# mlnoga/nightlight

Hardware: AMD Instinct MI355X
Metric: stacked Mpixels/sec (sigma-clip, 128x4096x4096 fp32) (higher is better)
Workload: dtype f32; 1 GPU; 128 x 4096x4096 fp32 frames, sigma-clip kappa=3, rows split over 1 GPU(s), frames resident in HBM; frames=128, width=4096, image_rows=4096, rows_per_gpu=4096, mode=2, preheat_steps=64, clip_low=6836157, clip_high=13270993

## Files before the change

### nightlight_amd/csrc/nlstack_internal.hpp

```cpp
#pragma once

#include <string.h>

#include <string>
#include <vector>

#include "background.hpp"
#include "dev_memory.hpp"
#include "stars.hpp"
#include "stack_kernels.h"

namespace nl {

extern thread_local std::string g_err;
int fail(int code, const char *fmt, ...);

int require_device(int *count = nullptr);
int select_device(int device);

template <class Run>
int with_scratch_handle(int width, int height, int device, Run run)
{
    nl_stack_t *h = nl_stack_create(1, width, height, 0, height, device);
    if (!h) return NL_ERR_HIP;
// ... 13 lines not shown
        hipError_t e_ = (call);                                                             \
        if (e_ != hipSuccess)                                                               \
            return fail(NL_ERR_HIP, "%s failed: %s (%s:%d)", #call, hipGetErrorString(e_), \
                        __FILE__, __LINE__);                                                \
    } while (0)

constexpr int kTimingRing = 64;
constexpr int kStageSlots = 4;
constexpr int kStatBlocks = 2048;
constexpr int kOrderRing = 8;
constexpr size_t kScratchBytes = sizeof(unsigned long long) * nl::kScratchWords;

struct nl_stack {
    int device = 0;
    int n_frames = 0, width = 0, height = 0, row0 = 0, rows = 0;
    int n_capacity = 0;
    int64_t npix = 0;
    int64_t fstride = 0;
    int64_t fstride_owned = 0;
    hipStream_t stream = nullptr;
    hipEvent_t ring_start[kTimingRing] = {}, ring_stop[kTimingRing] = {};
    hipEvent_t ring_dom0[kTimingRing] = {}, ring_dom1[kTimingRing] = {};
    bool ring_dom0_is_start[kTimingRing] = {};
    bool ring_timed[kTimingRing] = {};
    int64_t pass_seq = 0;
    int64_t copy_waits_pass = 0;
    hipEvent_t ev_start = nullptr, ev_stop = nullptr;
    hipEvent_t ev_dom0 = nullptr, ev_dom1 = nullptr;
    hipStream_t side_stream = nullptr;
    hipEvent_t ev_fork = nullptr, ev_join = nullptr;
    hipEvent_t ev_order[kOrderRing] = {};
    int order_seq = 0;
    unsigned ev_rel = 0;
    float *d_frames_owned = nullptr;
    float *d_frames = nullptr;
    float *d_out = nullptr;
    float *d_acc = nullptr;
    float *d_weights = nullptr;
    bool has_weights = false;
    float *d_xstat = nullptr;
    unsigned long long *d_sets = nullptr;
    int cur_set = 0;
    bool sets_clean = false;
    bool partial_clean = false;
    unsigned long long *d_partial = nullptr;
    float2 *d_bounds = nullptr;
    unsigned char *d_nrounds = nullptr;
    bool bounds_tried = false;
    unsigned fb_hint = 0;
    unsigned gen_hint = 0;
    bool last_weighted = false;
    bool last_fused = false;
    bool last_tail_fused = false;
    bool last_lists = false;
    unsigned dev_flags = 0;
    unsigned *d_fb_list = nullptr;
    unsigned *d_fb_count = nullptr;
    unsigned *d_gen_list = nullptr;
    bool force_exact = false;
    int exact_flavour = 0;
    bool last_used_fast = false;
    unsigned long long *d_counters = nullptr;
    unsigned long long *d_counters_own = nullptr;
    double *d_stat_partial = nullptr;
    unsigned *d_lf_list[2] = {nullptr, nullptr};
    uint4 *d_lf_state[2] = {nullptr, nullptr};
    unsigned *d_lf_count = nullptr;
    int lf_lanes = 0;
    bool lf_tried = false;
    nl::DevBuffer ingest;
    hipStream_t copy_stream = nullptr;
    size_t stage_cap[kStageSlots] = {0, 0, 0, 0};
    nl::DevBuffer ingest_async;
    double *d_stat_partial_async = nullptr;
    void *h_stage[kStageSlots] = {nullptr, nullptr, nullptr, nullptr};
    hipEvent_t stage_done[kStageSlots] = {nullptr, nullptr, nullptr, nullptr};
    bool stage_used[kStageSlots] = {false, false, false, false};
    int stage_next = 0;
    bool uploads_pending = false;
    struct FrameScratch {
        nl::ParkedBuffer bp_diff, bp_seg, bp_list;
        nl::DevBuffer bp_small;
        nl::DevBuffer cfa;
        nl::StarWork star_work;
        nl::BackWork back_work;
        size_t bytes() const
        {
            return bp_diff.bytes + bp_seg.bytes + bp_list.bytes + bp_small.bytes + cfa.bytes + star_work.bytes() +
                   back_work.bytes();
        }
        void release(int device)
        {
            bp_diff.release(device);
            bp_seg.release(device);
            bp_list.release(device);
            bp_small.release();
            cfa.release();
            star_work.release();
            back_work.release();
        }
    } frame_scratch;
    int max_grid = 0;
    int last_mode = -1;
    bool last_has_counters = false;
    bool pending = false;
    const char *last_kernel = "";
// ... 16 lines not shown
```

### nightlight_amd/csrc/nlstack_pass.hip

```cpp
#include <mutex>

#include "nlstack_internal.hpp"

namespace {

constexpr int kListGrid = 2048;
constexpr int kCoopGrid = 16384;
constexpr int kListLanes = 4;
constexpr unsigned kFusedMaxList = 512;
constexpr unsigned kTailFusedMaxList = 512;
constexpr const char *kWinsorPlanShallow = "1:6,1:12:4,0:0:4";
constexpr const char *kWinsorPlanDeep = "2:12,2:16:8,3:24:4,0:0:4";
constexpr int kWinsorCascadeMaxFrames = 96;

constexpr unsigned kDevPlainProtocol = 1u;
constexpr unsigned kDevReplayInFront = 2u;
constexpr unsigned kDevNoDecision = 4u;
constexpr unsigned kDevNoTile = 16u;
constexpr unsigned kDevUntimed = 32u;
constexpr unsigned kDevNoWinsorCascade = 128u;
constexpr unsigned kDevNoSharedHints = 512u;
constexpr unsigned kDevRemovedPasses = 1024u | 2048u;
constexpr unsigned kDevTwoStreamTail = 8192u;
constexpr unsigned kDevNoCertificate = 16384u;

struct HintKey { int frames; int64_t npix; int mode; bool weighted; };
struct HintEntry { HintKey key; unsigned fb, gen; };
std::mutex g_hint_mu;
std::vector<HintEntry> g_hints;
constexpr size_t kHintEntries = 32;

void hints_store(const HintKey &k, unsigned fb, unsigned gen)
{
    std::lock_guard<std::mutex> lk(g_hint_mu);
    for (HintEntry &e : g_hints)
        if (e.key.frames == k.frames && e.key.npix == k.npix && e.key.mode == k.mode && e.key.weighted == k.weighted) {
            e.fb = fb; e.gen = gen;
            return;
        }
    if (g_hints.size() >= kHintEntries) g_hints.erase(g_hints.begin());
    g_hints.push_back({k, fb, gen});
}

bool hints_load(const HintKey &k, unsigned *fb, unsigned *gen)
{
    std::lock_guard<std::mutex> lk(g_hint_mu);
    for (const HintEntry &e : g_hints)
        if (e.key.frames == k.frames && e.key.npix == k.npix && e.key.mode == k.mode && e.key.weighted == k.weighted) {
            *fb = e.fb; *gen = e.gen;
            return true;
        }
    return false;
}

int next_pow2(int n)
{
    int p = 1;
    while (p < n) p <<= 1;
    return p;
}

}

static int dense_grid(int64_t items, int64_t max_grid, int width, int pixels_per_item)
{
    int64_t g = items < max_grid ? items : max_grid;
    if (g <= 8 || items <= g) return (int)g;
    g &= ~(int64_t)7;
    auto gcd = [](int64_t x, int64_t y) { while (y) { const int64_t t = x % y; x = y; y = t; } return x; };
    const int64_t most = (int64_t)width / 64 > 8 * pixels_per_item ? (int64_t)width / 64 : 8 * pixels_per_item;
    for (int tries = 0; tries < 64 && g > 8 && gcd(g * pixels_per_item, (int64_t)width) > most; tries++) g -= 8;
    return (int)g;
}

extern "C" {

static const nl::LinfitCascade *linfit_cascade(nl_stack_t *h, nl::LinfitCascade *out)
// ... 31 lines not shown
    if (h->d_bounds) return true;
    if (h->bounds_tried) return false;
    h->bounds_tried = true;
    if (cached_malloc((void **)&h->d_bounds, (size_t)nl::kBoundRounds * (size_t)h->npix * sizeof(float2), h->device) != hipSuccess ||
        cached_malloc((void **)&h->d_nrounds, (size_t)h->npix, h->device) != hipSuccess) {
        (void)hipGetLastError();
        if (h->d_bounds) { (void)hipFree(h->d_bounds); h->d_bounds = nullptr; }
        h->d_nrounds = nullptr;
        return false;
    }
    return true;
}

static bool fused_protocol_on()
{
    static const bool on = [] { const char *e = getenv("NL_FUSED"); return !(e && e[0] == '0'); }();
    return on;
}

static int auto_select_mode(int l)
{
    if (l >= 25) return NL_ST_LINEAR_FIT;
    if (l >= 15) return NL_ST_WINSOR_SIGMA;
    if (l >= 6) return NL_ST_SIGMA;
    return NL_ST_MEAN;
}


enum class Engine {
    Mean,
    MedianRegisters,
    MedianMultiLane,
    Listed,
    SigmaFast,
    WeightedTile,
    DenseReplay,
    ExactColumns,
};

struct PassSetup {
    int mode;
    bool weighted;
    bool timed;
    bool fused;
    nl::StackArgs a;
};

struct PassFacts {
    bool has_counters = false;
    bool used_fast = false;
    bool lists = false;
    bool fused = false;
    bool tail_fused = false;
    bool zeroed_behind = false;
};

static void set_last_pass(nl_stack *h, const PassFacts &f)
{
    h->last_has_counters = f.has_counters;
    h->last_used_fast = f.used_fast;
    h->last_lists = f.lists;
    h->last_fused = f.fused;
    h->last_tail_fused = f.tail_fused;
    h->sets_clean = f.fused;
}

static Engine select_engine(const nl_stack *h, int mode, bool weighted, const nl::StackArgs &a)
{
    const bool fast = !h->force_exact;
    const int n = a.n_frames;
    if (mode == NL_ST_MEAN) return Engine::Mean;
    if (fast && mode == NL_ST_MEDIAN && nl::fast_supported(mode, weighted, n, a.npix)) return Engine::MedianRegisters;
    if (fast && mode == NL_ST_MEDIAN && nl::fast_ml_supported(mode, weighted, n, a.npix)) return Engine::MedianMultiLane;
    if (fast && h->d_fb_list &&
        (nl::mad_fast_supported(mode, weighted, n, a.npix) || (mode == NL_ST_MAD_SIGMA && nl::fast_ml_supported(mode, weighted, n, a.npix)) ||
         nl::linfit_ml_supported(mode, n, a.npix) || nl::linfit_fast_supported(mode, n, a.npix)))
        return Engine::Listed;
    if (fast && h->d_fb_list && (nl::fast_supported(mode, weighted, n, a.npix) || nl::fast_ml_supported(mode, weighted, n, a.npix)))
        return Engine::SigmaFast;
    if ((h->exact_flavour == 3 ||
         (fast && weighted && !(h->dev_flags & kDevNoTile) &&
          n <= (mode == NL_ST_WINSOR_SIGMA ? nl::kTileMaxFramesWinsor : nl::kTileMaxFramesSigma))) &&
        nl::tile_supported(mode, weighted, n))
        return Engine::WeightedTile;
    if ((h->exact_flavour == 2 || (fast && (weighted || n > 512))) && nl::coop_supported(mode, weighted, n))
        return Engine::DenseReplay;
    return Engine::ExactColumns;
}

static nl::FastArgs list_args(const nl_stack *h, bool exact_list, bool generic_list)
{
    nl::FastArgs f;
    memset(&f, 0, sizeof f);
    if (exact_list) {
        f.fb_list = h->d_fb_list;
        f.fb_count = h->d_fb_count;
        f.fb_capacity = (unsigned)h->npix;
    }
    if (generic_list) {
        f.gen_list = h->d_gen_list;
        f.gen_count = h->d_fb_count + 1;
        f.gen_capacity = (unsigned)h->npix;
    }
    return f;
}

static int replay_list(nl_stack *h, int mode, bool weighted, const nl::StackArgs &a)
{
    int lanes = 0;
    size_t lds = 0;
    if (nl::exact_plan(mode, weighted, a.n_frames, a.n_pad, kListLanes, &lanes, &lds) != 0)
        return fail(NL_ERR_TOO_MANY_FRAMES, "%d frames do not fit the per-pixel LDS column (mode %d)", a.n_frames, mode);
    nl::StackArgs e = a;
    e.list = h->d_fb_list;
    e.list_count = h->d_fb_count;
    e.list_capacity = (unsigned)h->npix;
// ... 117 lines not shown
        unsigned *base = reinterpret_cast<unsigned *>(cb.state[i]);
        f.cas_list[i] = base;
        f.cas_state[i] = base + 2 * (size_t)h->npix;
        f.cas_count[i] = cb.list[i];
    }
    f.cas_stages = pl.stages;
    for (int k = 0; k < pl.stages; k++) { f.cas_pass[k] = pl.pass[k]; f.cas_cap[k] = pl.cap[k]; f.cas_group[k] = pl.group[k]; }
    return true;
}

static int run_sigma_fast(nl_stack *h, const PassSetup &p, PassFacts *facts)
{
    const int mode = p.mode;
    nl::StackArgs a = p.a;
    if (mode == NL_ST_WINSOR_SIGMA && a.n_frames > 128 && fused_protocol_on() && ensure_bounds(h)) {
        a.bounds = h->d_bounds;
        a.nrounds = h->d_nrounds;
    }
    nl::FastArgs f = list_args(h, true, true);
    f.fb_snap = h->d_fb_count + 2;
    f.gen_hint = h->gen_hint;
    const bool cascade = mode == NL_ST_WINSOR_SIGMA && winsor_setup(h, a.n_frames, f);
    nl::StackArgs e = a;
    e.list = h->d_fb_list;
    e.list_count = h->d_fb_count;
    e.list_capacity = (unsigned)h->npix;
    const bool coop = nl::coop_supported(mode, p.weighted, a.n_frames) != 0;
    unsigned *snap = h->d_fb_count + 2;
    int grid0 = 0, grid1 = 0;
    replay_grids(h, &grid0, &grid1);
    struct Fork { nl_stack *h; nl::StackArgs e; int mode; unsigned *snap; int grid0; bool cascade; hipError_t err; } fork{h, e, mode, snap, grid0, cascade, hipSuccess};
    nl::AfterDominant after = nullptr;
    if (coop) after = [](void *u) {
        Fork *k = static_cast<Fork *>(u);
        nl_stack *hh = k->h;
        const char *ignored = "";
        const bool own = (hh->dev_flags & kDevUntimed) || k->cascade;
        hipEvent_t fork_ev = own ? hh->ev_fork : hh->ev_dom1;
        hipError_t err = own ? hipEventRecord(hh->ev_fork, hh->stream) : hipSuccess;
        const bool in_front = (hh->dev_flags & kDevReplayInFront) != 0;
        const hipStream_t s = in_front ? hh->stream : hh->side_stream;
        if (!in_front && err == hipSuccess) err = hipStreamWaitEvent(hh->side_stream, fork_ev, 0);
        nl::StackArgs first = k->e;
        first.list_snap = k->snap;
        first.list_part = 0;
        if (err == hipSuccess) err = nl::launch_stack_sigma_coop(k->mode, first, k->grid0, s, &ignored);
        if (err == hipSuccess) err = hipEventRecord(hh->ev_join, s);
        k->err = err;
    };
    static const bool tail_fused_on = [] { const char *e = getenv("NL_TAIL_FUSED"); return !(e && e[0] == '0'); }();
    const bool tail_fused = tail_fused_on && !(h->dev_flags & (kDevTwoStreamTail | kDevReplayInFront)) && p.fused && coop && !cascade &&
                            nl::tail_fused_supported(mode, p.weighted, a.n_frames) != 0 && h->fb_hint != 0 &&
                            h->fb_hint - 1u <= kTailFusedMaxList;
    nl::StackArgs first_replay = e;
    first_replay.list_snap = snap;
    first_replay.list_part = 0;
    unsigned replay_blocks = h->fb_hint + 31u;
    replay_blocks = replay_blocks < 64u ? 64u : replay_blocks > 768u ? 768u : replay_blocks;
    if (tail_fused) after = nullptr;
    if (a.n_frames <= 128)
        NL_HIP(nl::launch_stack_sigma_fast(a, f, h->stream, &h->last_kernel, p.timed ? h->ev_dom1 : nullptr,
                                           mode == NL_ST_WINSOR_SIGMA, after, &fork,
                                           tail_fused ? &first_replay : nullptr, replay_blocks));
    else
        NL_HIP(nl::launch_stack_sigma_ml(a, f, h->stream, &h->last_kernel, p.timed ? h->ev_dom1 : nullptr,
                                         mode == NL_ST_WINSOR_SIGMA, after, &fork));
    NL_HIP(fork.err);
    if (coop) {
        const char *exact_name = "";
        e.list_snap = snap;
        e.list_part = 1;
        NL_HIP(nl::launch_stack_sigma_coop(mode, e, grid1, h->stream, &exact_name));
        if (!tail_fused) NL_HIP(hipStreamWaitEvent(h->stream, h->ev_join, 0));
    } else {
        const int rc = replay_list(h, mode, p.weighted, a);
        if (rc != NL_OK) return rc;
    }
    if (!p.fused) {
        NL_HIP(nl::launch_reduce_counters(h->d_partial, nl::kClipSlots, h->d_counters, h->stream, h->d_fb_count, true));
        facts->zeroed_behind = true;
    }
    facts->has_counters = true;
    facts->used_fast = true;
    facts->lists = true;
    facts->fused = p.fused;
    facts->tail_fused = tail_fused;
    return NL_OK;
}

static int run_weighted_tile(nl_stack *h, const PassSetup &p, PassFacts *facts)
{
    const int64_t tiles = (p.a.npix + 63) / 64;
    const int64_t g = tiles < (1 << 20) ? tiles : (1 << 20);
    NL_HIP(nl::launch_stack_sigma_tile(p.mode, p.a, (int)g, h->stream, &h->last_kernel));
    NL_HIP(hipEventRecord(h->ev_dom1, h->stream));
    NL_HIP(nl::launch_reduce_counters(h->d_partial, nl::kClipSlots, h->d_counters, h->stream));
    facts->has_counters = true;
    return NL_OK;
}

static int run_dense_replay(nl_stack *h, const PassSetup &p, PassFacts *facts)
{
    nl::StackArgs a = p.a;
    const int rc = decision_pass(h, p, a);
    if (rc != NL_OK) return rc;
    const int per_item = p.mode == NL_ST_MEDIAN ? 1 : nl::coop_group(a);
    const int64_t items = a.npix / per_item;
    const int64_t most = 262144;
    const int g = dense_grid(items, most, h->width, per_item);
    if (p.mode == NL_ST_MEDIAN) NL_HIP(nl::launch_stack_median_coop(a, (int)g, h->stream, &h->last_kernel));
    else                        NL_HIP(nl::launch_stack_sigma_coop(p.mode, a, (int)g, h->stream, &h->last_kernel));
    NL_HIP(hipEventRecord(h->ev_dom1, h->stream));
    NL_HIP(nl::launch_reduce_counters(h->d_partial, nl::kClipSlots, h->d_counters, h->stream));
    facts->has_counters = p.mode != NL_ST_MEDIAN;
    return NL_OK;
}

static int run_exact_columns(nl_stack *h, const PassSetup &p, PassFacts *facts)
{
    nl::StackArgs a = p.a;
    int lanes = 0;
    size_t lds = 0;
    if (nl::exact_plan(p.mode, p.weighted, a.n_frames, a.n_pad, 64, &lanes, &lds) != 0)
        return fail(NL_ERR_TOO_MANY_FRAMES, "%d frames do not fit the per-pixel LDS column (mode %d)", a.n_frames, p.mode);
    a.tiles = (a.npix + lanes - 1) / lanes;
    const int grid = (int)(a.tiles < (int64_t)h->max_grid ? a.tiles : (int64_t)h->max_grid);
    NL_HIP(nl::launch_stack_exact(p.mode, p.weighted, a, lanes, grid, lds, h->stream, &h->last_kernel));
    NL_HIP(hipEventRecord(h->ev_dom1, h->stream));
    NL_HIP(nl::launch_reduce_counters(h->d_partial, nl::kClipSlots, h->d_counters, h->stream));
    facts->has_counters = p.mode != NL_ST_MEDIAN;
    return NL_OK;
}

static int run_async_impl(nl_stack_t *h, int mode, float sigma_low, float sigma_high, float ref_loc);

int nl_stack_run_async(nl_stack_t *h, int mode, float sigma_low, float sigma_high, float ref_loc)
{
    const int rc = run_async_impl(h, mode, sigma_low, sigma_high, ref_loc);
    if (rc != NL_OK && h && h->stream) {
// ... 139 lines not shown
    if (hipSetDevice(h->device) != hipSuccess || hipEventSynchronize(to) != hipSuccess ||
        hipEventElapsedTime(&ms, from, to) != hipSuccess)
        return -1.0f;
    return ms;
}

float nl_stack_last_dominant_kernel_ms(nl_stack_t *h) { return h && h->ev_dom0 ? elapsed_ms(h, h->ev_dom0, h->ev_dom1) : -1.0f; }

int nl_stack_set_exact(nl_stack_t *h, int on)
{
    NL_CHECK_HANDLE(h);
    if (on < 0 || on > 4) return fail(NL_ERR_INVALID_ARG, "set_exact: unknown flavour %d (0 ... 4)", on);
    if (on == 4)
        return fail(NL_ERR_INVALID_ARG, "set_exact: flavour 4 (four pixels per wave) was removed with the experiments build");
    h->force_exact = on != 0;
    h->exact_flavour = on;
    return NL_OK;
}

int nl_stack_set_dev_flags(nl_stack_t *h, unsigned flags)
{
    NL_CHECK_HANDLE(h);
    if (flags & kDevRemovedPasses)
        return fail(NL_ERR_INVALID_ARG, "set_dev_flags: switches 1024 / 2048 (split / persistent LDS-column pass) were removed with the "
                                        "experiments build");
    h->dev_flags = flags;
    return NL_OK;
}

static int64_t last_list_length(nl_stack_t *h, int which)
{
    if (hipSetDevice(h->device) != hipSuccess) return -1;
    if (h->last_lists) {
        unsigned long long c = 0;
        if (hipMemcpyAsync(&c, h->d_counters + 2, sizeof c, hipMemcpyDeviceToHost, h->stream) != hipSuccess) return -1;
        if (hipStreamSynchronize(h->stream) != hipSuccess) return -1;
        return which == 0 ? (int64_t)(c & 0xffffffffull) : (int64_t)(c >> 32);
    }
    unsigned c = 0;
    if (hipMemcpyAsync(&c, h->d_fb_count + which, sizeof c, hipMemcpyDeviceToHost, h->stream) != hipSuccess) return -1;
    if (hipStreamSynchronize(h->stream) != hipSuccess) return -1;
    return (int64_t)c;
}

int64_t nl_stack_last_fallback_pixels(nl_stack_t *h)
{
    if (!h || !h->last_used_fast || !h->d_fb_count) return 0;
    return last_list_length(h, 0);
}

int nl_stack_last_pass_protocol(nl_stack_t *h)
{
    if (!h) return 0;
    return (h->last_fused ? 1 : 0) | (h->last_tail_fused ? 2 : 0);
}

int64_t nl_stack_last_generic_pixels(nl_stack_t *h)
{
    if (!h || !h->last_used_fast || !h->d_fb_count || !h->d_gen_list) return 0;
    return last_list_length(h, 1);
}

int nl_stack_linfit_stage_counts(nl_stack_t *h, unsigned *counts, int n)
{
    if (!h || !counts || n <= 0 || !h->d_lf_count || h->last_mode != NL_ST_LINEAR_FIT || !h->last_used_fast) return 0;
    if (hipSetDevice(h->device) != hipSuccess) return -1;
    unsigned c[nl::kLinfitCounters] = {};
    if (hipMemcpyAsync(c, h->d_lf_count, sizeof c, hipMemcpyDeviceToHost, h->stream) != hipSuccess) return -1;
    if (hipStreamSynchronize(h->stream) != hipSuccess) return -1;
    const int m = n < nl::kLinfitCounters ? n : nl::kLinfitCounters;
    for (int i = 0; i < m; i++) counts[i] = c[i];
    return m;
}

int nl_stack_pass_times(nl_stack_t *h, int back, float *pass_ms, float *dominant_ms)
{
    NL_CHECK_HANDLE(h);
    if (back < 0 || back >= kTimingRing || (int64_t)back >= h->pass_seq)
        return fail(NL_ERR_INVALID_ARG, "pass_times: pass %d back is not in the ring of %d", back, kTimingRing);
    const int slot = (int)((h->pass_seq - 1 - back) % kTimingRing);
    if (!h->ring_timed[slot])
        return fail(NL_ERR_INVALID_ARG, "pass_times: pass %d back ran without timing events (developer switch 32)", back);
    NL_HIP(hipEventSynchronize(h->ring_stop[slot]));
    float ms = -1.0f;
    if (pass_ms) {
        NL_HIP(hipEventElapsedTime(&ms, h->ring_start[slot], h->ring_stop[slot]));
        *pass_ms = ms;
    }
    if (dominant_ms) {
        NL_HIP(hipEventElapsedTime(&ms, h->ring_dom0_is_start[slot] ? h->ring_start[slot] : h->ring_dom0[slot], h->ring_dom1[slot]));
        *dominant_ms = ms;
    }
    return NL_OK;
}

int nl_stack_copy_counters_async(nl_stack_t *h, void *device_dst)
{
    NL_CHECK_HANDLE(h);
    if (!device_dst) return fail(NL_ERR_INVALID_ARG, "copy_counters_async: null destination");
    if (h->last_has_counters)
        NL_HIP(hipMemcpyAsync(device_dst, h->d_counters, 2 * sizeof(unsigned long long), hipMemcpyDeviceToDevice, h->stream));
    else
        NL_HIP(hipMemsetAsync(device_dst, 0, 2 * sizeof(unsigned long long), h->stream));
    return NL_OK;
}

void *nl_stack_stream(nl_stack_t *h) { return h ? (void *)h->stream : nullptr; }
// ... 100 lines not shown
```

### nightlight_amd/csrc/stack_exact_coop_impl.hpp

```cpp
#pragma once
#include <stdint.h>

#include "stack_kernels.h"

#ifndef NL_T0
#define NL_T0() do {} while (0)
#define NL_T(slot) do {} while (0)
#define NL_TDECL() do {} while (0)
#define NL_TFLUSH() do {} while (0)
#endif

namespace nl {

namespace {

__device__ __forceinline__ float sqrt_like_go(float x)
{
    return (float)__builtin_sqrt((double)x);
}

__device__ __forceinline__ unsigned long long ballot64(bool p)
{
    return __builtin_amdgcn_ballot_w64(p);
}
// ... 199 lines not shown
            nl += __popcll(ml);
            nr += __popcll(mr);
        }
        lds_fence();
        const int pairs = min(nl, nr);
        int s_cnt = 0;
        for (int base = 0; base < pairs; base += 64) {
            const int i = base + lane;
            const bool ok = i < pairs && (int)lpos[i] < (int)rfwd[nr - 1 - i];
            const unsigned long long m = ballot64(ok);
            s_cnt += __popcll(m);
            if (m != ~0ull) break;
        }
        for (int base = 0; base < s_cnt; base += 64) {
            const int i = base + lane;
            if (i < s_cnt) {
                const int pl = (int)lpos[i], pr = (int)rfwd[nr - 1 - i];
                const float xl = a[pl], xr = a[pr];
                a[pl] = xr;
                a[pr] = xl;
            }
        }
        const int r_next = s_cnt < nr ? (int)rfwd[nr - 1 - s_cnt] : -1;
        const int l_prev = s_cnt > 0 ? (int)lpos[s_cnt - 1] : -1;
        const int r = max(r_next, l_prev);
        lds_fence();
        const int offset = r - left + 1;
        if (k <= offset) {
            right = r;
        } else {
            left = r + 1;
            k -= offset;
        }
    }
    return a[left];
}

__device__ float coop_select_median(float *a, unsigned short *lpos, unsigned short *rfwd, int n)
{
    const int k = (n >> 1) + 1;
    const float upper = coop_select(a, lpos, rfwd, n, k);
    if (n & 1) return upper;
    const int lane = threadIdx.x;
    float lower = -__builtin_inff();
    for (int base = 0; base < k - 1; base += 64) {
        const int idx = base + lane;
        if (idx < k - 1) lower = fmaxf(lower, a[idx]);
    }
#pragma unroll
    for (int o = 32; o > 0; o >>= 1) lower = fmaxf(lower, __shfl_xor(lower, o, 64));
    return 0.5f * (lower + upper);
}

}

template <bool WINSOR, bool W, int GROUP, int PF = 2>
__device__ __forceinline__ void coop_body(const StackArgs &p, float *a, const unsigned block, const unsigned nblocks)
{
    float *wz = a + p.n_frames;
    float *wt = a + (WINSOR ? 2 : 1) * p.n_frames;
    unsigned short *lpos = reinterpret_cast<unsigned short *>(a + ((WINSOR ? 2 : 1) + (W ? 1 : 0)) * p.n_frames);
    unsigned short *rfwd = lpos + p.n_frames;
    const int lane = threadIdx.x;
    const int N = p.n_frames;
    int64_t limit = p.npix;
    if (p.list) {
        const unsigned cnt = __atomic_load_n(p.list_count, __ATOMIC_RELAXED);
        limit = cnt < p.list_capacity ? cnt : p.list_capacity;
    }
    long long c_lo = 0, c_hi = 0;
    NL_TDECL();

    int64_t first = 0;
    if (p.list && p.list_snap) {
        unsigned s = 0;
        if (lane == 0) {
            s = __atomic_load_n(p.list_snap, __ATOMIC_RELAXED);
            if (s == 0u) {
                s = atomicCAS(p.list_snap, 0u, (unsigned)limit + 1u);
                if (s == 0u) s = (unsigned)limit + 1u;
            }
        }
        s = (unsigned)__shfl((int)s, 0, 64);
        const int64_t snap = min((int64_t)(s - 1u), limit);
        if (p.list_part == 0) limit = snap; else first = snap;
    }
    int64_t wg = block;
    if (!p.list && (nblocks & 7u) == 0u) wg = (int64_t)(block & 7u) * (nblocks >> 3) + (block >> 3);
    static_assert(PF == 2 || GROUP == 4, "deep register prefetch is for the whole-tile replays");
    const bool dense = p.list == nullptr;
    float wreg[PF] = {};
    if constexpr (W) {
#pragma unroll
        for (int c = 0; c < PF; c++) wreg[c] = c * 64 + lane < N ? p.weights[c * 64 + lane] : 0.0f;
    }
    if constexpr (GROUP > 1) limit = p.npix / GROUP;
    for (int64_t item = first + wg; item < limit; item += nblocks) {
      float4 grp[PF];
      if constexpr (GROUP > 1) {
        static_assert(GROUP == 4, "one 16-byte load per lane and chunk");
#pragma unroll
        for (int c = 0; c < PF; c++) {
            const int k = min(c * 64 + lane, N - 1);
            grp[c] = *reinterpret_cast<const float4 *>(p.frames + item * GROUP + (int64_t)k * p.stride);
        }
      }
// ... 121 lines not shown
                        int nf = 0;
                        for (int base = m & ~63; base < n; base += 64) {
                            const int idx = base + lane;
                            const bool in = idx >= m && idx < n;
                            const float x = in ? a[idx] : 0.0f;
                            const bool fill = in && !(x < lo || x > hi);
                            const unsigned long long mf = ballot64(fill);
                            if (fill) rfwd[nf + below64(mf)] = (unsigned short)idx;
                            nf += __popcll(mf);
                        }
                        lds_fence();
                        int nh = 0;
                        for (int base = 0; base < m; base += 64) {
                            const int idx = base + lane;
                            const float x = idx < m ? a[idx] : 0.0f;
                            const bool hole = idx < m && (x < lo || x > hi);
                            const unsigned long long mh = ballot64(hole);
                            if (hole) {
                                const int src = (int)rfwd[nf - 1 - (nh + below64(mh))];
                                a[idx] = a[src];
                                if (W) wt[idx] = wt[src];
                            }
                            nh += __popcll(mh);
                        }
                        lds_fence();
                        n = m;
                    }
                }
                NL_T(3);
                if (n == before || n <= 1) {
                    res = mean;
                    if constexpr (W) {
                        float sw, ws;
                        seq_sum2(n, [&](int i) { return i < n ? a[i] * wt[i] : 0.0f; },
                                 [&](int i) { return i < n ? wt[i] : 0.0f; }, sw, ws);
                        res = sw / ws;
                    }
                    break;
                }
            }
        }
        if (lane == 0) p.out[pix] = res;
        NL_T(4);
      }
    }
    NL_TFLUSH();
    if (lane == 0) {
        unsigned long long *slot = p.final ? p.final : p.partial + 2 * (size_t)(block % kClipSlots);
        if (c_lo) atomicAdd(slot + 0, (unsigned long long)c_lo);
        if (c_hi) atomicAdd(slot + 1, (unsigned long long)c_hi);
        if (p.final && p.list && p.list_part == 1 && block == 0)
            p.final[2] = (unsigned long long)p.list_count[0] | ((unsigned long long)p.list_count[1] << 32);
    }
}

}
```

### nightlight_amd/csrc/stack_fast_mlg.hip

```cpp
#include "fast_ml_common.hpp"

namespace nl {

#ifdef NL_ROUND_STATS
__device__ unsigned long long nl_dbg_rounds_mlg[8];
extern "C" int nl_debug_round_stats_mlg(unsigned long long *out, int reset)
{
    if (hipMemcpyFromSymbol(out, HIP_SYMBOL(nl_dbg_rounds_mlg), sizeof(unsigned long long) * 8) != hipSuccess) return -1;
    if (reset) {
        unsigned long long z[8] = {};
        if (hipMemcpyToSymbol(HIP_SYMBOL(nl_dbg_rounds_mlg), z, sizeof(z)) != hipSuccess) return -1;
    }
    return 0;
}
#define NL_STAT(i, x) atomicAdd(&nl_dbg_rounds_mlg[i], (unsigned long long)(x))
#else
#define NL_STAT(i, x) ((void)0)
#endif

}
#include "stack_fast_mlg_impl.hpp"
#include "launch_common.hpp"
namespace nl {

template <int LPP, bool WINSOR>
__global__ __launch_bounds__(64) __attribute__((amdgpu_waves_per_eu(1, 2)))
void stack_sigma_mlg_kernel(StackArgs p, FastArgs q)
{
    mlg_body<LPP, WINSOR>(p, q, blockIdx.x, gridDim.x);
}

hipError_t launch_stack_sigma_mlg(const StackArgs &args, const FastArgs &fargs, unsigned grid, hipStream_t stream,
                                  bool winsor)
{
    Launcher L(stream);
    with_bool(winsor, [&](auto W) {
        constexpr bool WINSOR = decltype(W)::value;
        if (args.n_frames <= kMlNS)
            L(stack_sigma_mlg_kernel<1, WINSOR>, grid, 64, 0, args, fargs);
        else
            with_ml_lanes(args.n_frames, [&](auto LPP) {
                L(stack_sigma_mlg_kernel<decltype(LPP)::value, WINSOR>, grid, 64, 0, args, fargs);
            });
    });
    return L.err;
}

}
```

### nightlight_amd/csrc/stack_fast_mlg_impl.hpp

```cpp
#pragma once
#include "fast_ml_common.hpp"

namespace nl {

namespace {

template <int LPP>
struct MlgLayout {
    static constexpr int NS = kMlNS, NT = NS * LPP;
    static constexpr int PW = 64 / LPP;
    static constexpr int G = NT / 4;
    static constexpr int X = 0, P1 = NT, P2 = P1 + G + 1, ROWS = P2 + G + 1;
    static constexpr int ROUNDINGS = NS + 20;
};

__device__ __forceinline__ void lds_settle_g() { asm volatile("s_waitcnt lgkmcnt(0)" ::: "memory"); }

template <int PW, bool COARSE>
__device__ __forceinline__ int walk_up(const float *x, int j, int lim, float thr, bool on, int top)
{
    if (COARSE) {
        bool more = on;
        while (__any(more)) {
            int t = 0;
            static_range<0, 8>([&](auto S) NL_INL {
                const int idx = j + 8 * decltype(S)::value + 7;
                const float val = x[min(idx, top) * PW];
                t += (idx < lim && val < thr) ? 1 : 0;
            });
            if (more) { j += 8 * t; more = t == 8; }
        }
    }
    bool more = on;
    while (__any(more)) {
        int t = 0;
        static_range<0, 8>([&](auto I) NL_INL {
            const int idx = j + decltype(I)::value;
            const float val = x[min(idx, top) * PW];
            t += (idx < lim && val < thr) ? 1 : 0;
        });
        if (more) { j += t; more = t == 8; }
    }
    return j;
}

template <int PW, bool COARSE>
__device__ __forceinline__ int walk_down(const float *x, int j, int lim, float thr, bool on)
{
    if (COARSE) {
        bool more = on;
        while (__any(more)) {
            int t = 0;
            static_range<0, 8>([&](auto S) NL_INL {
                const int idx = j - 8 * decltype(S)::value - 8;
                const float val = x[max(idx, 0) * PW];
                t += (idx >= lim && val > thr) ? 1 : 0;
            });
            if (more) { j -= 8 * t; more = t == 8; }
        }
    }
    bool more = on;
    while (__any(more)) {
        int t = 0;
        static_range<0, 8>([&](auto I) NL_INL {
            const int idx = j - 1 - decltype(I)::value;
            const float val = x[max(idx, 0) * PW];
            t += (idx >= lim && val > thr) ? 1 : 0;
        });
        if (more) { j -= t; more = t == 8; }
    }
    return j;
}

template <class LY>
__device__ __forceinline__ void range_moments(const float *col, float c, int i, int j, int top, float &d, float &q,
                                              float &pmag)
{
    constexpr int PW = LY::PW;
    const int gi = (i + 3) >> 2, gj = j >> 2;
    const bool tabled = gi <= gj;
    const float p1i = col[(LY::P1 + gi) * PW], p1j = col[(LY::P1 + gj) * PW];
    const float p2i = col[(LY::P2 + gi) * PW], p2j = col[(LY::P2 + gj) * PW];
    const int lo_end = tabled ? 4 * gi : j;
    const int hi_beg = tabled ? 4 * gj : j;
    float dp = 0.0f, qp = 0.0f;
    static_range<0, 3>([&](auto U) NL_INL {
        constexpr int u = decltype(U)::value;
        const int kl = i + u, kh = j - 1 - u;
        const float xl = col[(LY::X + min(kl, top)) * PW], xh = col[(LY::X + max(kh, 0)) * PW];
        const float e = (kl < lo_end) ? xl - c : 0.0f;
        const float f = (kh >= hi_beg) ? xh - c : 0.0f;
        dp += e; qp = __builtin_fmaf(e, e, qp);
        dp += f; qp = __builtin_fmaf(f, f, qp);
    });
    d = dp + (tabled ? p1j - p1i : 0.0f);
    q = qp + (tabled ? p2j - p2i : 0.0f);
    pmag = (tabled ? p2j : 0.0f) + qp;
}

}

template <int LPP, bool WINSOR>
__device__ __forceinline__ void mlg_body(const StackArgs &p, const FastArgs &q, const unsigned block, const unsigned nblocks)
{
    using LY = MlgLayout<LPP>;
    constexpr int NS = LY::NS, NT = LY::NT, PW = LY::PW;
    __shared__ float lds[LY::ROWS * PW];
    if (q.in_list) { fused_collect_slots(p, block); snapshot_fb_list(q); }

    const int lane = threadIdx.x & 63;
    const int role = threadIdx.x % LPP;
    float *col = lds + threadIdx.x / LPP;
    constexpr int top = NT - 1;
    constexpr float kErrF = (float)(2 * LY::ROUNDINGS + 8);

    int c_lo_total = 0, c_hi_total = 0;
    const int64_t limit = q.in_list ? (int64_t)min(*q.in_count, q.in_capacity) : p.npix;
    const int64_t sweep = (int64_t)nblocks * PW;

    for (int64_t wg_item = (int64_t)block * PW; wg_item < limit; wg_item += sweep) {
        int N = p.n_frames;
        asm volatile("" : "+s"(N));
        const int64_t item = wg_item + threadIdx.x / LPP;
        const bool on = item < limit;
        int64_t pix = item;
        if (q.in_list) pix = on ? (int64_t)q.in_list[item] : 0;

#ifdef NL_ROUND_STATS
        const unsigned long long t0 = __builtin_readcyclecounter();
#endif
        float v[NS];
        int n;
        if constexpr (LPP == 1) n = gather_sorted<NS, NS>(p.frames, p.stride, N, (unsigned)(on ? pix : 0) * 4u, v);
        else                    n = ml_gather_sorted<LPP, NS, false>(p.frames, p.stride, N, on, pix, role, v);

#ifdef NL_ROUND_STATS
        asm volatile("s_waitcnt vmcnt(0) lgkmcnt(0)" ::: "memory");
        const unsigned long long t1 = __builtin_readcyclecounter();
#endif
        {
            float *mine = col + (LY::X + role * NS) * PW;
            static_range<0, NS>([&](auto K) NL_INL { mine[decltype(K)::value * PW] = v[decltype(K)::value]; });
        }
        lds_settle_g();
        bool active = on && n > 0;
        bool to_exact = false;
        const float c = col[(LY::X + min(max(n >> 1, 0), top)) * PW];

        {
            float d0 = 0, d1 = 0, d2 = 0, d3 = 0, q0 = 0, q1 = 0, q2 = 0, q3 = 0;
            static_chunks<0, NS / 4, 4>([&](auto K) NL_INL {
                constexpr int k = 4 * decltype(K)::value;
                const float e0 = v[k] - c, e1 = v[k + 1] - c, e2 = v[k + 2] - c, e3 = v[k + 3] - c;
                d0 += e0; d1 += e1; d2 += e2; d3 += e3;
                q0 = __builtin_fmaf(e0, e0, q0); q1 = __builtin_fmaf(e1, e1, q1);
                q2 = __builtin_fmaf(e2, e2, q2); q3 = __builtin_fmaf(e3, e3, q3);
            });
            const float t1 = (d0 + d1) + (d2 + d3), t2 = (q0 + q1) + (q2 + q3);
            float o1 = 0.0f, o2 = 0.0f;
            if constexpr (LPP > 1) {
                const float a1 = dpp_f<kSwap1>(t1), a2 = dpp_f<kSwap1>(t2);
                if constexpr (LPP == 2) {
                    o1 = (role & 1) ? a1 : 0.0f;
                    o2 = (role & 1) ? a2 : 0.0f;
                } else {
                    const float pair1 = t1 + a1, pair2 = t2 + a2;
                    const float b1 = dpp_f<kSwap2>(pair1), b2 = dpp_f<kSwap2>(pair2);
                    o1 = ((role & 1) ? a1 : 0.0f) + ((role & 2) ? b1 : 0.0f);
                    o2 = ((role & 1) ? a2 : 0.0f) + ((role & 2) ? b2 : 0.0f);
                }
            }
            float *m1 = col + (LY::P1 + role * (NS / 4)) * PW, *m2 = col + (LY::P2 + role * (NS / 4)) * PW;
            float s1 = o1, s2 = o2;
            static_range<0, NS / 4>([&](auto G) NL_INL {
                constexpr int g = decltype(G)::value;
                m1[g * PW] = s1;
                m2[g * PW] = s2;
                static_range<0, 4>([&](auto U) NL_INL {
                    const float e = v[4 * g + decltype(U)::value] - c;
                    s1 += e;
                    s2 = __builtin_fmaf(e, e, s2);
                });
            });
            if (role == LPP - 1) {
                m1[(NS / 4) * PW] = s1;
                m2[(NS / 4) * PW] = s2;
            }
        }
        lds_settle_g();

#ifdef NL_ROUND_STATS
        const unsigned long long t2 = __builtin_readcyclecounter();
#endif
        float res = p.ref_loc;
        int c_lo = 0, c_hi = 0;
        int a = 0, b = n;
        const float *x = col + LY::X * PW;

        if (lane == 0) NL_STAT(4, 1);
        while (__any(active)) {
            if (lane == 0) NL_STAT(2, 1);
            if (active && role == 0) NL_STAT(3, 1);
            const int cnt = b - a;
            const float fcnt = (float)cnt;
            const float inv_cnt = 1.0f / fcnt;
            const int kk = min(max(a + (cnt >> 1), 0), top);
            const float upper = x[kk * PW], lower = x[max(kk - 1, 0) * PW];
            const float median = (cnt & 1) ? upper : 0.5f * (lower + upper);
            const float xmin = x[min(max(a, 0), top) * PW], xmax = x[min(max(b - 1, 0), top) * PW];

            float dsum, qsum, pmag;
            range_moments<LY>(col, c, a, b, top, dsum, qsum, pmag);
            const float delta = dsum * inv_cnt;
            const float m = c + delta;
            const float aa = qsum * inv_cnt;
            const float bb = delta * delta;
            const float var = fmaxf(aa - bb, 0.0f);
            const float mag = pmag * inv_cnt * ((float)b * inv_cnt) + bb;

            const float amax = fmaxf(fabsf(xmin), fabsf(xmax));
            const float err_o = kErrF * kU * mag;
            const float eps_r = 1.02f * (fcnt + 8.0f) * kU;
            const float e_m = 1.02f * (fcnt + 2.0f) * kU * amax;
            const float v_up = var + err_o;
            const float v_dn = fmaxf(var - err_o, 0.0f);
            const float v_hi = v_up + v_up * eps_r + e_m * e_m;
            const float v_lo = fmaxf(v_dn - v_dn * eps_r, 0.0f);
            float s_max = __fsqrt_rn(v_hi) * (1.0f + 4.0f * kU);
            float s_min = __fsqrt_rn(v_lo) * (1.0f - 4.0f * kU);
            bool bail = !(v_hi < 3.0e38f);

            if constexpr (WINSOR) {
                WinsorInterval wi;
                wi.start(s_min, s_max, q.gen_round_cap > 0 ? q.gen_round_cap : 100);
                bool inner = active && !bail;
                int jl = a, jh = b;
                bool first = true;
                while (__any(inner)) {
                    if (lane == 0) NL_STAT(0, 1);
// ... 107 lines not shown
```

### nightlight_amd/csrc/stack_kernels.h

```cpp
#pragma once
#include <hip/hip_runtime.h>
#include <stddef.h>
#include <stdint.h>

#include "../../include/nlstack.h"

#if defined(__HIPCC__)
#ifdef NL_PLAIN_STORES
#define NL_STORE_RESULT(ptr, val) (*(ptr) = (val))
#else
#define NL_STORE_RESULT(ptr, val) __builtin_nontemporal_store((val), (ptr))
#endif
#endif

namespace nl {

constexpr size_t kLdsBudgetBytes = 160 * 1024;
constexpr int kClipSlots = 256;

struct StackArgs {
    const float *frames;
    int64_t stride;
    int64_t npix;
    int64_t tiles;
    int n_frames;
    int n_pad;
    const float *weights;
    const float *xstat;
    float sig_lo, sig_hi, ref_loc;
    float *out;
    unsigned long long *partial;
    const unsigned *list;
    const unsigned *list_count;
    unsigned list_capacity;
    unsigned *list_snap;
    int list_part;
    unsigned long long *final;
    unsigned long long *zero_next;
    float2 *bounds;
    unsigned char *nrounds;
};

constexpr int kScratchWords = 2 * kClipSlots + 2;

struct FastArgs {
    unsigned *fb_list;
    unsigned *fb_count;
    unsigned fb_capacity;
    unsigned *fb_snap;
    unsigned *gen_list;
    unsigned *gen_count;
    unsigned gen_capacity;
    unsigned gen_hint;
    const unsigned *in_list;
    const unsigned *in_count;
    unsigned in_capacity;
    unsigned *cas_list[2];
    unsigned *cas_state[2];
    unsigned *cas_count[2];
    int cas_stages;
    int cas_pass[6], cas_cap[6];
    int cas_group[6];
    unsigned *cont_list;
    unsigned *cont_state;
    unsigned *cont_count;
    unsigned cont_region;
    const unsigned *in_state;
    unsigned in_region, in_regions, in_group;
    int pass_budget, round_cap;
    int record_only = 0;
    int cert_first = 0, cert_every = 1;
    int gen_round_cap = 0;
};

void set_last_error(const char *msg);

struct SigmaBisection {
    float low_left = 1.0f, low_right = 11.0f, low_mid;
    float high_left = 1.0f, high_right = 11.0f, high_mid;
    float perc_low, perc_high, total;
    int i = 0;
    SigmaBisection(float clip_perc_low, float clip_perc_high, int64_t total_samples)
        : perc_low(clip_perc_low), perc_high(clip_perc_high), total((float)total_samples)
    {
        low_mid = 0.5f * (low_left + low_right);
        high_mid = 0.5f * (high_left + high_right);
    }
    bool step(int64_t clip_low, int64_t clip_high)
    {
        const float pl = (float)clip_low * 100.0f / total;
        const float ph = (float)clip_high * 100.0f / total;
        const int delta_l = (int)(100 * pl + 0.5f) - (int)(100 * perc_low);
        const int delta_h = (int)(100 * ph + 0.5f) - (int)(100 * perc_high);
        if ((delta_l == 0 && delta_h == 0) || i >= 20) return true;
        i++;
        if (delta_l > 0) { low_left = low_mid; low_mid = 0.5f * (low_left + low_right); }
        else if (delta_l < 0) { low_right = low_mid; low_mid = 0.5f * (low_left + low_right); }
        if (delta_h > 0) { high_left = high_mid; high_mid = 0.5f * (high_left + high_right); }
        else if (delta_h < 0) { high_right = high_mid; high_mid = 0.5f * (high_left + high_right); }
        return false;
    }
};

struct SigmaNewton {
    float sig_low = 6.0f, sig_high = 6.0f;
    const float epsilon = 0.005f;
    float perc_low, total;
    int i = 0, phase = 0;
    float delta_l = 0, delta_h = 0, new_low = 0;
    int64_t base_lo = 0, base_hi = 0;
    SigmaNewton(float clip_perc_low, int64_t total_samples) : perc_low(clip_perc_low), total((float)total_samples) {}
    float next_low() const { return phase == 1 ? sig_low + epsilon : sig_low; }
    float next_high() const { return phase == 2 ? sig_high + epsilon : sig_high; }
    int step(int64_t clip_low, int64_t clip_high)
    {
        if (phase == 0) {
            base_lo = clip_low; base_hi = clip_high;
            const float pl = (float)clip_low * 100.0f / total, ph = (float)clip_high * 100.0f / total;
            delta_l = pl - perc_low;
            delta_h = ph - perc_low;
            const int li = (int)(100 * delta_l + 0.5f), hi = (int)(100 * delta_h + 0.5f);
            if ((li == 0 && hi == 0) || i >= 20) return 1;
            i++; phase = 1;
            return 0;
        }
// ... 122 lines not shown
```

Baseline: 10720 Mpixels/s.

## Fold counter reduction into exact coop tail and compact generic prefix tables

```diff
diff --git a/nightlight_amd/csrc/nlstack_internal.hpp b/nightlight_amd/csrc/nlstack_internal.hpp
--- a/nightlight_amd/csrc/nlstack_internal.hpp
+++ b/nightlight_amd/csrc/nlstack_internal.hpp
@@ -89,6 +89,7 @@
     bool last_weighted = false;
     bool last_fused = false;
     bool last_tail_fused = false;
+    bool last_lean_tail = false;
     bool last_lists = false;
     unsigned dev_flags = 0;
     unsigned *d_fb_list = nullptr;
diff --git a/nightlight_amd/csrc/nlstack_pass.hip b/nightlight_amd/csrc/nlstack_pass.hip
--- a/nightlight_amd/csrc/nlstack_pass.hip
+++ b/nightlight_amd/csrc/nlstack_pass.hip
@@ -23,6 +23,7 @@
 constexpr unsigned kDevRemovedPasses = 1024u | 2048u;
 constexpr unsigned kDevTwoStreamTail = 8192u;
 constexpr unsigned kDevNoCertificate = 16384u;
+constexpr unsigned kDevWideTail = 32768u;
 
 struct HintKey { int frames; int64_t npix; int mode; bool weighted; };
 struct HintEntry { HintKey key; unsigned fb, gen; };
@@ -160,6 +161,7 @@
     bool lists = false;
     bool fused = false;
     bool tail_fused = false;
+    bool lean_tail = false;
     bool zeroed_behind = false;
 };
 
@@ -170,6 +172,7 @@
     h->last_lists = f.lists;
     h->last_fused = f.fused;
     h->last_tail_fused = f.tail_fused;
+    h->last_lean_tail = f.lean_tail;
     h->sets_clean = f.fused;
 }
 
@@ -393,6 +396,9 @@
     const bool tail_fused = tail_fused_on && !(h->dev_flags & (kDevTwoStreamTail | kDevReplayInFront)) && p.fused && coop && !cascade &&
                             nl::tail_fused_supported(mode, p.weighted, a.n_frames) != 0 && h->fb_hint != 0 &&
                             h->fb_hint - 1u <= kTailFusedMaxList;
+    const bool lean_tail = !p.fused && coop && !cascade && nl::tail_fused_supported(mode, p.weighted, a.n_frames) != 0 &&
+                           !(h->dev_flags & (kDevWideTail | kDevPlainProtocol));
+    f.gen_compact = lean_tail ? 1 : 0;
     nl::StackArgs first_replay = e;
     first_replay.list_snap = snap;
     first_replay.list_part = 0;
@@ -411,14 +417,18 @@
         const char *exact_name = "";
         e.list_snap = snap;
         e.list_part = 1;
+        if (lean_tail) {
+            e.book = h->d_counters;
+            NL_HIP(hipStreamWaitEvent(h->stream, h->ev_join, 0));
+        }
         NL_HIP(nl::launch_stack_sigma_coop(mode, e, grid1, h->stream, &exact_name));
-        if (!tail_fused) NL_HIP(hipStreamWaitEvent(h->stream, h->ev_join, 0));
+        if (!tail_fused && !lean_tail) NL_HIP(hipStreamWaitEvent(h->stream, h->ev_join, 0));
     } else {
         const int rc = replay_list(h, mode, p.weighted, a);
         if (rc != NL_OK) return rc;
     }
     if (!p.fused) {
-        NL_HIP(nl::launch_reduce_counters(h->d_partial, nl::kClipSlots, h->d_counters, h->stream, h->d_fb_count, true));
+        if (!lean_tail) NL_HIP(nl::launch_reduce_counters(h->d_partial, nl::kClipSlots, h->d_counters, h->stream, h->d_fb_count, true));
         facts->zeroed_behind = true;
     }
     facts->has_counters = true;
@@ -426,6 +436,7 @@
     facts->lists = true;
     facts->fused = p.fused;
     facts->tail_fused = tail_fused;
+    facts->lean_tail = lean_tail;
     return NL_OK;
 }
 
@@ -671,7 +682,7 @@
 int nl_stack_last_pass_protocol(nl_stack_t *h)
 {
     if (!h) return 0;
-    return (h->last_fused ? 1 : 0) | (h->last_tail_fused ? 2 : 0);
+    return (h->last_fused ? 1 : 0) | (h->last_tail_fused ? 2 : 0) | (h->last_lean_tail ? 4 : 0);
 }
 
 int64_t nl_stack_last_generic_pixels(nl_stack_t *h)
diff --git a/nightlight_amd/csrc/stack_exact_coop_impl.hpp b/nightlight_amd/csrc/stack_exact_coop_impl.hpp
--- a/nightlight_amd/csrc/stack_exact_coop_impl.hpp
+++ b/nightlight_amd/csrc/stack_exact_coop_impl.hpp
@@ -275,6 +275,39 @@
     return 0.5f * (lower + upper);
 }
 
+}
+
+__device__ __forceinline__ void book_counters(const StackArgs &p, const unsigned nblocks)
+{
+    const int lane = threadIdx.x;
+    unsigned *words = reinterpret_cast<unsigned *>(p.partial + 2 * kClipSlots);
+    unsigned ticket = 0;
+    if (lane == 0) {
+        __atomic_thread_fence(__ATOMIC_RELEASE);
+        ticket = atomicAdd(words + 3, 1u);
+        __atomic_thread_fence(__ATOMIC_ACQUIRE);
+    }
+    ticket = (unsigned)__shfl((int)ticket, 0, 64);
+    if (ticket != nblocks - 1u) return;
+    __atomic_thread_fence(__ATOMIC_ACQUIRE);
+    unsigned long long lo = 0, hi = 0;
+    for (int i = lane; i < kClipSlots; i += 64) {
+        lo += __hip_atomic_load(p.partial + 2 * (size_t)i, __ATOMIC_RELAXED, __HIP_MEMORY_SCOPE_AGENT);
+        hi += __hip_atomic_load(p.partial + 2 * (size_t)i + 1, __ATOMIC_RELAXED, __HIP_MEMORY_SCOPE_AGENT);
+    }
+#pragma unroll
+    for (int o = 32; o > 0; o >>= 1) {
+        lo += ((unsigned long long)(unsigned)__shfl_xor((int)(lo >> 32), o, 64) << 32) | (unsigned)__shfl_xor((int)lo, o, 64);
+        hi += ((unsigned long long)(unsigned)__shfl_xor((int)(hi >> 32), o, 64) << 32) | (unsigned)__shfl_xor((int)hi, o, 64);
+    }
+    if (lane == 0) {
+        const unsigned fb = __hip_atomic_load(words + 0, __ATOMIC_RELAXED, __HIP_MEMORY_SCOPE_AGENT);
+        const unsigned gen = __hip_atomic_load(words + 1, __ATOMIC_RELAXED, __HIP_MEMORY_SCOPE_AGENT);
+        p.book[0] = lo;
+        p.book[1] = hi;
+        p.book[2] = (unsigned long long)fb | ((unsigned long long)gen << 32);
+    }
+    for (int i = lane; i < kScratchWords; i += 64) p.partial[i] = 0ull;
 }
 
 template <bool WINSOR, bool W, int GROUP, int PF = 2>
@@ -502,6 +535,7 @@
         if (p.final && p.list && p.list_part == 1 && block == 0)
             p.final[2] = (unsigned long long)p.list_count[0] | ((unsigned long long)p.list_count[1] << 32);
     }
-}
-
-}
+    if (p.book) book_counters(p, nblocks);
+}
+
+}
diff --git a/nightlight_amd/csrc/stack_fast_mlg.hip b/nightlight_amd/csrc/stack_fast_mlg.hip
--- a/nightlight_amd/csrc/stack_fast_mlg.hip
+++ b/nightlight_amd/csrc/stack_fast_mlg.hip
@@ -23,12 +23,14 @@
 #include "launch_common.hpp"
 namespace nl {
 
-template <int LPP, bool WINSOR>
+template <int LPP, bool WINSOR, int TS = 4>
 __global__ __launch_bounds__(64) __attribute__((amdgpu_waves_per_eu(1, 2)))
 void stack_sigma_mlg_kernel(StackArgs p, FastArgs q)
 {
-    mlg_body<LPP, WINSOR>(p, q, blockIdx.x, gridDim.x);
+    mlg_body<LPP, WINSOR, TS>(p, q, blockIdx.x, gridDim.x);
 }
+
+constexpr int kCompactStride = 16;
 
 hipError_t launch_stack_sigma_mlg(const StackArgs &args, const FastArgs &fargs, unsigned grid, hipStream_t stream,
                                   bool winsor)
@@ -36,7 +38,9 @@
     Launcher L(stream);
     with_bool(winsor, [&](auto W) {
         constexpr bool WINSOR = decltype(W)::value;
-        if (args.n_frames <= kMlNS)
+        if (!WINSOR && args.n_frames <= kMlNS && fargs.gen_compact)
+            L(stack_sigma_mlg_kernel<1, false, kCompactStride>, grid, 64, 0, args, fargs);
+        else if (args.n_frames <= kMlNS)
             L(stack_sigma_mlg_kernel<1, WINSOR>, grid, 64, 0, args, fargs);
         else
             with_ml_lanes(args.n_frames, [&](auto LPP) {
diff --git a/nightlight_amd/csrc/stack_fast_mlg_impl.hpp b/nightlight_amd/csrc/stack_fast_mlg_impl.hpp
--- a/nightlight_amd/csrc/stack_fast_mlg_impl.hpp
+++ b/nightlight_amd/csrc/stack_fast_mlg_impl.hpp
@@ -5,12 +5,15 @@
 
 namespace {
 
-template <int LPP>
+template <int LPP, int TS = 4>
 struct MlgLayout {
+    static_assert(TS == 4 || (LPP == 1 && TS % 4 == 0 && kMlNS % TS == 0), "compact tables: one lane per pixel");
     static constexpr int NS = kMlNS, NT = NS * LPP;
     static constexpr int PW = 64 / LPP;
-    static constexpr int G = NT / 4;
-    static constexpr int X = 0, P1 = NT, P2 = P1 + G + 1, ROWS = P2 + G + 1;
+    static constexpr int STRIDE = TS;
+    static constexpr int Z = TS == 4 ? 1 : 0;
+    static constexpr int G = NT / TS;
+    static constexpr int X = 0, P1 = NT, P2 = P1 + G + Z, ROWS = P2 + G + Z;
     static constexpr int ROUNDINGS = NS + 20;
 };
 
@@ -73,14 +76,39 @@
 }
 
 template <class LY>
+__device__ __forceinline__ void prefix_entry(const float *col, float c, int g4, int top, float &p1, float &p2)
+{
+    constexpr int PW = LY::PW;
+    if constexpr (LY::STRIDE == 4) {
+        p1 = col[(LY::P1 + g4) * PW];
+        p2 = col[(LY::P2 + g4) * PW];
+    } else {
+        constexpr int R = LY::STRIDE / 4;
+        const int e = g4 / R, left = 4 * (g4 - e * R);
+        const float t1 = col[(LY::P1 + max(e - 1, 0)) * PW], t2 = col[(LY::P2 + max(e - 1, 0)) * PW];
+        float s1 = e > 0 ? t1 : 0.0f, s2 = e > 0 ? t2 : 0.0f;
+        static_range<0, 4 * (R - 1)>([&](auto T) NL_INL {
+            constexpr int t = decltype(T)::value;
+            const float d = col[(LY::X + min(e * LY::STRIDE + t, top)) * PW] - c;
+            const float n1 = s1 + d, n2 = __builtin_fmaf(d, d, s2);
+            s1 = t < left ? n1 : s1;
+            s2 = t < left ? n2 : s2;
+        });
+        p1 = s1;
+        p2 = s2;
+    }
+}
+
+template <class LY>
 __device__ __forceinline__ void range_moments(const float *col, float c, int i, int j, int top, float &d, float &q,
                                               float &pmag)
 {
     constexpr int PW = LY::PW;
     const int gi = (i + 3) >> 2, gj = j >> 2;
     const bool tabled = gi <= gj;
-    const float p1i = col[(LY::P1 + gi) * PW], p1j = col[(LY::P1 + gj) * PW];
-    const float p2i = col[(LY::P2 + gi) * PW], p2j = col[(LY::P2 + gj) * PW];
+    float p1i, p2i, p1j, p2j;
+    prefix_entry<LY>(col, c, gi, top, p1i, p2i);
+    prefix_entry<LY>(col, c, gj, top, p1j, p2j);
     const int lo_end = tabled ? 4 * gi : j;
     const int hi_beg = tabled ? 4 * gj : j;
     float dp = 0.0f, qp = 0.0f;
@@ -100,10 +128,10 @@
 
 }
 
-template <int LPP, bool WINSOR>
+template <int LPP, bool WINSOR, int TS = 4>
 __device__ __forceinline__ void mlg_body(const StackArgs &p, const FastArgs &q, const unsigned block, const unsigned nblocks)
 {
-    using LY = MlgLayout<LPP>;
+    using LY = MlgLayout<LPP, TS>;
     constexpr int NS = LY::NS, NT = LY::NT, PW = LY::PW;
     __shared__ float lds[LY::ROWS * PW];
     if (q.in_list) { fused_collect_slots(p, block); snapshot_fb_list(q); }
@@ -170,12 +198,15 @@
                     o2 = ((role & 1) ? a2 : 0.0f) + ((role & 2) ? b2 : 0.0f);
                 }
             }
-            float *m1 = col + (LY::P1 + role * (NS / 4)) * PW, *m2 = col + (LY::P2 + role * (NS / 4)) * PW;
+            constexpr int R = LY::STRIDE / 4;
+            float *m1 = col + (LY::P1 + role * (NS / 4) - (1 - LY::Z)) * PW, *m2 = col + (LY::P2 + role * (NS / 4) - (1 - LY::Z)) * PW;
             float s1 = o1, s2 = o2;
             static_range<0, NS / 4>([&](auto G) NL_INL {
                 constexpr int g = decltype(G)::value;
-                m1[g * PW] = s1;
-                m2[g * PW] = s2;
+                if constexpr (g % R == 0 && (LY::Z || g > 0)) {
+                    m1[g / R * PW] = s1;
+                    m2[g / R * PW] = s2;
+                }
                 static_range<0, 4>([&](auto U) NL_INL {
                     const float e = v[4 * g + decltype(U)::value] - c;
                     s1 += e;
@@ -183,8 +214,8 @@
                 });
             });
             if (role == LPP - 1) {
-                m1[(NS / 4) * PW] = s1;
-                m2[(NS / 4) * PW] = s2;
+                m1[(NS / 4) / R * PW] = s1;
+                m2[(NS / 4) / R * PW] = s2;
             }
         }
         lds_settle_g();
diff --git a/nightlight_amd/csrc/stack_kernels.h b/nightlight_amd/csrc/stack_kernels.h
--- a/nightlight_amd/csrc/stack_kernels.h
+++ b/nightlight_amd/csrc/stack_kernels.h
@@ -39,6 +39,7 @@
     unsigned long long *zero_next;
     float2 *bounds;
     unsigned char *nrounds;
+    unsigned long long *book;
 };
 
 constexpr int kScratchWords = 2 * kClipSlots + 2;
@@ -71,6 +72,7 @@
     int record_only = 0;
     int cert_first = 0, cert_every = 1;
     int gen_round_cap = 0;
+    int gen_compact = 0;
 };
 
 void set_last_error(const char *msg);
```

Result: slower. 10470 Mpixels/s (-2.3%).
